# SokhengDin/DNN-MPPI-MPC

Hardware: NVIDIA B200
Metric: mppi_sample_steps_per_sec (higher is better)
Workload: dtype f32

## Files before the change

dnn-mppi-mpc_b200/csrc/mppi_api.cu:

```cuda
#include <cuda_runtime.h>
#include <dlfcn.h>
#include <nccl.h>

#include <algorithm>
#include <cmath>
#include <cstdio>
#include <cstdlib>
#include <cstring>
#include <string>
#include <vector>

#include "mppi_device.cuh"
#include "mppi_launch.h"
#include "mppi_mlp.h"

namespace {

struct NcclApi {
    void *lib = nullptr;
    ncclResult_t (*GetUniqueId)(ncclUniqueId *) = nullptr;
    ncclResult_t (*CommInitRank)(ncclComm_t *, int, ncclUniqueId, int) = nullptr;
    ncclResult_t (*AllGather)(const void *, void *, size_t, ncclDataType_t, ncclComm_t, cudaStream_t) = nullptr;
    ncclResult_t (*CommDestroy)(ncclComm_t) = nullptr;
    const char *(*GetErrorString)(ncclResult_t) = nullptr;
// ... 263 lines not shown
    CKC(cudaSetDevice(c.device));
    cudaDeviceProp prop;
    CKC(cudaGetDeviceProperties(&prop, c.device));
    h->n_sm = prop.multiProcessorCount;
    CKC(cudaStreamCreateWithFlags(&h->stream, cudaStreamNonBlocking));
    h->own_stream = true;

    const int R = c.n_robots, T = c.T, K = c.K;
    int min_cta = 128;
    if (const char *env = std::getenv("MPPI_MIN_CTA_SAMPLES")) min_cta = std::max(32, std::min(MPPI_BLOCK, std::atoi(env)));
    const int chunks = (K + min_cta - 1) / min_cta;
    const int tick_model = (c.model == MPPI_MODEL_DIFFDRIVE_MLP) ? MPPI_MODEL_DIFFDRIVE : c.model;
    h->occ = std::max(1, mppi_tick_occupancy(tick_model, c.collision, c.cost_kind, h->sum, false, c.window, T, false));
    const int occ_stash = mppi_tick_occupancy(tick_model, c.collision, c.cost_kind, h->sum, false, c.window, T, true);
    h->stash = occ_stash >= MPPI_STASH_BLOCKS && c.model != MPPI_MODEL_DIFFDRIVE_MLP;
    int gx = (h->n_sm * h->occ + R - 1) / R;
    gx = std::max(1, std::min(gx, chunks));
    h->grid_x = gx;
    int gxs = (h->n_sm * std::max(1, occ_stash) + R - 1) / R;
    h->grid_x_stash = std::max(1, std::min(gxs, chunks));
    gx = std::max(h->grid_x, h->grid_x_stash);
    {
        const int occ_tpar = (h->sum && c.cost_kind == MPPI_COSTKIND_PATH && c.window != 20 && c.model != MPPI_MODEL_DIFFDRIVE_MLP)
                                 ? mppi_tick_occupancy(tick_model, c.collision, c.cost_kind, true, false, c.window, T, 2) : 0;
        const int gt = std::max(1, std::min(h->n_sm * std::max(1, occ_tpar), (K + 7) / 8));
        const bool fits = occ_tpar >= 1 && (K + gt - 1) / gt <= MPPI_TPAR_SLOTS;
        bool want = R == 1;
        if (const char *env = std::getenv("MPPI_TPAR")) want = std::atoi(env) != 0;
        if (std::getenv("MPPI_VERBOSE"))
            std::fprintf(stderr, "mppi_create: time-parallel rollout: occ %d grid %d fits %d want %d (stash %d sum %d window %d K %d T %d)\n",
                         occ_tpar, gt, (int)fits, (int)want, (int)h->stash, (int)h->sum, c.window, K, T);
        if (want && fits) {
            h->tpar = true;
            h->grid_x_tpar = gt;
            gx = std::max(gx, gt);
        }
        if (std::getenv("MPPI_VERBOSE"))
            std::fprintf(stderr, "mppi_create: rollout path %s, %d CTAs per robot\n", h->tpar ? "tpar" : h->stash ? "stash" : "regenerate",
                         h->tpar ? h->grid_x_tpar : h->stash ? h->grid_x_stash : h->grid_x);
    }

    CKC(gmalloc(h, &h->d_U, sizeof(float) * R * T * 2));
    CKC(cudaMemset(h->d_U, 0, sizeof(float) * R * T * 2));
    CKC(gmalloc(h, &h->d_M, sizeof(float) * T * T));
    CKC(gmalloc(h, &h->d_S, sizeof(float) * (size_t)R * K));
    CKC(gmalloc(h, &h->d_NC, sizeof(int) * (size_t)K));
    const int gmax = (gx + MPPI_MERGE_GROUP_CTAS - 1) / MPPI_MERGE_GROUP_CTAS;
    CKC(gmalloc(h, &h->d_part, sizeof(float) * (size_t)R * (gx + gmax) * MPPI_NF(T)));
    CKC(gmalloc(h, &h->d_out, sizeof(float) * (size_t)R * MPPI_OUT_STRIDE));
    CKC(cudaMemset(h->d_out, 0, sizeof(float) * (size_t)R * MPPI_OUT_STRIDE));
    CKC(gmalloc(h, &h->d_idx, sizeof(int) * R));
    CKC(cudaMemset(h->d_idx, 0, sizeof(int) * R));
    CKC(gmalloc(h, &h->d_ticket, sizeof(unsigned) * (size_t)R * (1 + gmax)));
    CKC(cudaMemset(h->d_ticket, 0, sizeof(unsigned) * (size_t)R * (1 + gmax)));
    CKC(cudaHostAlloc(&h->h_out, sizeof(float) * MPPI_OUT_STRIDE, cudaHostAllocMapped));
    std::memset(h->h_out, 0, sizeof(float) * MPPI_OUT_STRIDE);
    CKC(cudaHostGetDevicePointer(&h->h_out_dev, h->h_out, 0));
    CKC(gmalloc(h, &h->d_first, sizeof(unsigned long long)));
    CKC(cudaHostAlloc(&h->h_first, sizeof(unsigned long long), cudaHostAllocDefault));
    h->idx_mirror = 0; h->idx_mirror_ok = true;
    for (auto &e : h->ev) CKC(cudaEventCreate(&e));
    std::vector<float> M;
    build_filter(T, c.filter_kind, M);
    CKC(cudaMemcpy(h->d_M, M.data(), sizeof(float) * T * T, cudaMemcpyHostToDevice));

    TickArgs &a = h->args;
    std::memset(&a, 0, sizeof(a));
    a.K = K; a.T = T; a.window = c.window; a.yaw_wrap = c.yaw_wrap; a.clamp_nominal = c.clamp_nominal;
    a.k_offset = c.k_offset;
    {
        const double thr = (1.0 - c.param_exploration) * (double)c.K_global;
        long long n = (long long)std::ceil(thr);
        n = std::max(0LL, std::min((long long)c.K_global, n));
        a.n_exploit = (int)n;
    }
    a.dt = (float)c.dt; a.dt_over_L = (float)(c.dt / c.wheel_base);
    a.umax0 = (float)c.u_max[0]; a.umax1 = (float)c.u_max[1];
    for (int i = 0; i < 4; ++i) { a.sw[i] = (float)c.stage_w[i]; a.tw[i] = (float)c.term_w[i]; }
    const double gamma = c.param_lambda * (1.0 - c.param_alpha);
    a.use_gamma = gamma != 0.0;
    a.gq[0] = (float)(gamma * c.sigma[3] / det); a.gq[1] = (float)(-gamma * c.sigma[1] / det);
    a.gq[2] = (float)(-gamma * c.sigma[2] / det); a.gq[3] = (float)(gamma * c.sigma[0] / det);
    const double l00 = std::sqrt(c.sigma[0]), l10 = c.sigma[2] / l00;
    a.chol[0] = (float)l00; a.chol[1] = (float)l10; a.chol[2] = (float)std::sqrt(c.sigma[3] - l10 * l10);
    a.inv_temp = (float)(1.0 / c.temperature);
    for (int i = 0; i < 4; ++i) a.goal[i] = (float)c.goal[i];
    a.ctrl_w[0] = (float)c.ctrl_w[0]; a.ctrl_w[1] = (float)c.ctrl_w[1];
    a.soft_w = (float)c.soft_obs_weight; a.soft_sd = (float)c.soft_obs_safety;
    refresh_obstacle_args(h, nullptr, 0);
    a.U = h->d_U; a.idx = h->d_idx; a.M = h->d_M; a.part = h->d_part; a.ticket = h->d_ticket;
    a.part2 = h->d_part + (size_t)R * gx * MPPI_NF(T); a.ticket2 = h->d_ticket + R; a.merge_gmax = gmax;
    a.out = h->d_out; a.out_host = h->h_out_dev;
    if (c.model == MPPI_MODEL_DIFFDRIVE_MLP) {
        h->mlp = mlp_create(K, T);
        if (!h->mlp) { mppi_destroy(h); return MPPI_E_CUDA; }
    }
#undef CKC
    *out = h;
    return MPPI_OK;
}

int mppi_destroy(mppi_handle_t h) {
    if (!h) return MPPI_E_BADARG;
    cudaSetDevice(h->cfg.device);
    if (h->stream) cudaStreamSynchronize(h->stream);
    if (h->comm && g_nccl.CommDestroy) g_nccl.CommDestroy(h->comm);
    if (h->p2p)
        for (int p = 0; p < h->world; ++p)
            if (p != h->rank && h->peer_buf[p]) cudaIpcCloseMemHandle(h->peer_buf[p]);
    gfree(h, h->d_xchg); gfree(h, h->d_trace); gfree(h, h->d_loop);
    if (h->loop_graph) cudaGraphExecDestroy(h->loop_graph);
    if (h->cap_stream) cudaStreamDestroy(h->cap_stream);
    gfree(h, h->d_paths); gfree(h, h->d_path_len);
    gfree(h, h->d_Sc); gfree(h, h->d_Ssorted); gfree(h, h->d_sorted_idx); gfree(h, h->d_iota); gfree(h, h->d_sort_temp);
    if (h->mlp) mlp_destroy(h->mlp);
    gfree(h, h->d_path); gfree(h, h->d_U); gfree(h, h->d_M); gfree(h, h->d_S); gfree(h, h->d_part);
    gfree(h, h->d_out); gfree(h, h->d_idx); gfree(h, h->d_NC); gfree(h, h->d_ticket); gfree(h, h->d_first);
    gfree(h, h->d_bp_n); gfree(h, h->d_bp_s); gfree(h, h->d_send); gfree(h, h->d_recv); gfree(h, h->d_x0); gfree(h, h->d_opt); gfree(h, h->d_plant_log);
    if (h->h_out) cudaFreeHost(h->h_out);
    if (h->h_first) cudaFreeHost(h->h_first);
    if (h->h_bp_pack) cudaFreeHost(h->h_bp_pack);
    gfree(h, h->d_bp_pack);
    for (auto &e : h->ev) if (e) cudaEventDestroy(e);
    if (h->own_stream && h->stream) cudaStreamDestroy(h->stream);
    delete h;
    return MPPI_OK;
}

int mppi_set_stream(mppi_handle_t h, void *st) {
    if (!h) return MPPI_E_BADARG;
    if (h->own_stream && h->stream) { cudaStreamSynchronize(h->stream); cudaStreamDestroy(h->stream); }
    h->stream = (cudaStream_t)st;
    h->own_stream = false;
    return MPPI_OK;
}

int mppi_synchronize(mppi_handle_t h) {
    if (!h) return MPPI_E_BADARG;
    CK(h, cudaStreamSynchronize(h->stream));
    return check_tick_faults(h);
}

int mppi_set_ref_path(mppi_handle_t h, const double *path, int32_t n, int32_t ncol) {
    if (!h || !path || n < 1 || (ncol != 3 && ncol != 4)) return MPPI_E_BADARG;
    if (h->cfg.model == MPPI_MODEL_BICYCLE && ncol != 4) return fail(h, MPPI_E_BADARG, "bicycle model needs (N,4) path");
    if (h->cfg.cost_kind != MPPI_COSTKIND_PATH) return fail(h, MPPI_E_STATE, "goal / target cost kinds take no reference path");
    CK(h, cudaSetDevice(h->cfg.device));
    CK(h, cudaStreamSynchronize(h->stream));
    std::vector<float4> p((size_t)n);
    for (int i = 0; i < n; ++i) {
        const double *r = path + (size_t)i * ncol;
        p[i] = make_float4((float)r[0], (float)r[1], (float)r[2], ncol == 4 ? (float)r[3] : 0.f);
    }
    gfree(h, h->d_path); h->d_path = nullptr;
    gfree(h, h->d_bp_n); gfree(h, h->d_bp_s); h->d_bp_n = nullptr; h->d_bp_s = nullptr;
    CK(h, gmalloc(h, &h->d_path, sizeof(float4) * n));
    CK(h, cudaMemcpy(h->d_path, p.data(), sizeof(float4) * n, cudaMemcpyHostToDevice));
    CK(h, gmalloc(h, &h->d_bp_n, sizeof(unsigned) * (n + 2)));
    CK(h, gmalloc(h, &h->d_bp_s, sizeof(int) * (n + 2)));
    if (h->strict) {
        gfree(h, h->d_bp_pack); h->d_bp_pack = nullptr;
        if (h->h_bp_pack) { cudaFreeHost(h->h_bp_pack); h->h_bp_pack = nullptr; }
        h->bp_cap = n + 2;
        const size_t bytes = sizeof(unsigned long long) + (sizeof(unsigned) + sizeof(int)) * (size_t)h->bp_cap;
        CK(h, gmalloc(h, &h->d_bp_pack, bytes));
        CK(h, cudaHostAlloc(&h->h_bp_pack, bytes, cudaHostAllocDefault));
    }
// ... 696 lines not shown
```

dnn-mppi-mpc_b200/csrc/mppi_device.cuh:

```cuda
#pragma once
#include <cuda_runtime.h>
#include <stdint.h>
#include <math_constants.h>
#include "../../include/mppi_b200.h"

#ifndef MPPI_DEBUG_CHECKS
#define MPPI_DEBUG_CHECKS 0
#endif
#if MPPI_DEBUG_CHECKS
#include <assert.h>
#define MPPI_DCHECK(c) assert(c)
#else
#define MPPI_DCHECK(c) ((void)0)
#endif
#ifndef MPPI_BLOCK
#define MPPI_BLOCK 256
#endif
#define MPPI_WARPS (MPPI_BLOCK / 32)
#ifndef MPPI_SPT
#define MPPI_SPT 1
#endif
#define MPPI_CHUNK (MPPI_BLOCK * MPPI_SPT)
#ifndef MPPI_MIN_BLOCKS
#define MPPI_MIN_BLOCKS (MPPI_BLOCK >= 512 ? 1 : 768 / MPPI_BLOCK)
#endif
#define MPPI_STASH_BLOCKS (MPPI_BLOCK >= 512 ? 1 : 512 / MPPI_BLOCK)
#define MPPI_PENALTY 1.0e10f
#define MPPI_SENTINEL 1.0e18f
#define MPPI_OUT_HDR 12
#define MPPI_OUT_PEER_TIMEOUT 7
#define MPPI_OUT_FAULT 10
#define MPPI_OUT_STRIDE (MPPI_OUT_HDR + 8 * MPPI_MAX_T)
#define MPPI_OUT_UPRE (MPPI_OUT_HDR + 4 * MPPI_MAX_T)
#define MPPI_OUT_UOLD (MPPI_OUT_HDR + 6 * MPPI_MAX_T)
#define MPPI_NF(T) (4 + 2 * (T))
#define MPPI_MERGE_GROUP_CTAS 16
#define MPPI_NF_MAX MPPI_NF(MPPI_MAX_T)
#define MPPI_XCHG_SLOT(par, r) (((par) * MPPI_MAX_PEERS + (r)) * MPPI_NF_MAX)
#define MPPI_XCHG_WORDS (2 * MPPI_MAX_PEERS * MPPI_NF_MAX)
#define MPPI_XCHG_TRACE 8
#define MPPI_XCHG_BARRIER (MPPI_XCHG_WORDS + MPPI_XCHG_TRACE)
#define MPPI_XCHG_TOTAL (MPPI_XCHG_BARRIER + MPPI_MAX_PEERS)

enum : int {
    F_WRITE_S = 1,
    F_UPDATE = 2,
    F_FROM_S = 4,
    F_HOST_IDX = 8,
    F_TRIPLE_OUT = 16,
    F_KEEP_IDX = 32,
    F_IDX_ONLY = 64,
    F_P2P = 128,
    F_COST_SUM = 0x10000
};

struct TickArgs {
    int K, T, window, n_path, n_obs, yaw_wrap, use_gamma, clamp_nominal;
    int k_offset, n_exploit;
    float dt, dt_over_L, umax0, umax1;
    float sw[4], tw[4];
    float gq[4];
    float chol[3];
    float inv_temp;
    float obs_x[MPPI_MAX_OBSTACLES], obs_y[MPPI_MAX_OBSTACLES];
    float obs_r2[MPPI_MAX_OBSTACLES];
    float obs_far2[MPPI_MAX_OBSTACLES];
    float fp_hl, fp_hw;
    float goal[4];
    float ctrl_w[2];
    float soft_w, soft_sd;
    float obs_vx[MPPI_MAX_OBSTACLES], obs_vy[MPPI_MAX_OBSTACLES];
    float x0[4];
    uint32_t seed_lo, seed_hi, tick;
    int idx_host, flags;
    const float4 *path;
    const int *path_len;
    int path_stride;
    const float *x0_dev;
    float *U;
    int *idx;
    const float *M;
    const float *eps;
    float *S;
    int *NC;
    float *S_user;
    float *part;
    unsigned *ticket;
    float *part2;
    unsigned *ticket2;
    int merge_gmax;
    float *out;
    float *out_host;
    float *u0_out;
    float *triple_out;
    float *plant_state;
    float *plant_log;
    int plant_mode, plant_tick, plant_n;
    unsigned *loop_state;
    unsigned *loop_ticket;
    unsigned long long *peer_buf[MPPI_MAX_PEERS];
    int p2p_rank, p2p_world;
    unsigned p2p_seq;
    unsigned p2p_timeout_ms;
    unsigned long long *trace;
};

__device__ __forceinline__ void philox4x32_10(uint32_t &c0, uint32_t &c1, uint32_t &c2, uint32_t &c3,
                                              uint32_t k0, uint32_t k1) {
#pragma unroll
    for (int r = 0; r < 10; ++r) {
        const uint32_t h0 = __umulhi(0xD2511F53u, c0), l0 = 0xD2511F53u * c0;
        const uint32_t h1 = __umulhi(0xCD9E8D57u, c2), l1 = 0xCD9E8D57u * c2;
        c0 = h1 ^ c1 ^ k0; c1 = l1;
        c2 = h0 ^ c3 ^ k1; c3 = l0;
        k0 += 0x9E3779B9u; k1 += 0xBB67AE85u;
    }
}

__device__ __forceinline__ float u01_open(uint32_t r) {
    return __fadd_rn(__uint_as_float(0x3f800000u | (r >> 9)), -0.99999994f);
}

__device__ __forceinline__ void box_muller(uint32_t ra, uint32_t rb, float &z0, float &z1) {
    const float ua = u01_open(ra), ub = u01_open(rb);
    float rad;
    asm("sqrt.approx.ftz.f32 %0, %1;" : "=f"(rad) : "f"(__fmul_rn(-1.3862943611198906f, __log2f(ua))));
    const float ang = __fmul_rn(6.2831853071795865f, __fadd_rn(ub, -0.5f));
    z0 = __fmul_rn(rad, __cosf(ang));
    z1 = __fmul_rn(rad, __sinf(ang));
}

__device__ __forceinline__ void philox_eps_pair(const TickArgs &a, uint32_t k, uint32_t p, uint32_t robot, float e[4], uint32_t tick_add = 0u) {
    uint32_t c0 = k, c1 = p, c2 = a.tick + tick_add, c3 = robot;
    philox4x32_10(c0, c1, c2, c3, a.seed_lo, a.seed_hi);
    float z0, z1, z2, z3;
    box_muller(c0, c1, z0, z1);
    box_muller(c2, c3, z2, z3);
    e[0] = __fmul_rn(a.chol[0], z0);
    e[1] = __fmaf_rn(a.chol[1], z0, __fmul_rn(a.chol[2], z1));
    e[2] = __fmul_rn(a.chol[0], z2);
    e[3] = __fmaf_rn(a.chol[1], z2, __fmul_rn(a.chol[2], z3));
}

#ifndef MPPI_KEYIDX_SMEM
#define MPPI_KEYIDX_SMEM 1
#endif
struct TickSmem {
    float2 U[MPPI_MAX_T];
    float2 Q[MPPI_MAX_T];
    __align__(16) float wx[MPPI_MAX_WINDOW];
    __align__(16) float wy[MPPI_MAX_WINDOW];
    float2 wyv[MPPI_MAX_WINDOW];
    float x0[4];
    int win_start, n_win16;
    float4 cb[MPPI_MAX_WINDOW / 16];
    __align__(16) float ex[20];
    __align__(16) float ey[20];
    __align__(16) float ec[20];
    float c2x, c2y;
#if MPPI_KEYIDX_SMEM
    __align__(16) float kidx[20];
#endif
};

__device__ __forceinline__ void fill_window_expanded(TickSmem &sm, int nw, int tid, int nthreads) {
    const int jc = nw > 10 ? 10 : nw - 1;
    const float cx = -sm.wx[jc], cy = -sm.wy[jc];
    for (int j = tid; j < 20; j += nthreads) {
        const float wx = __fsub_rn(-sm.wx[j], cx), wy = __fsub_rn(-sm.wy[j], cy);
        const bool valid = j < nw;
        sm.ex[j] = valid ? wx : 0.f;
        sm.ey[j] = valid ? wy : 0.f;
        sm.ec[j] = valid ? __fmaf_rn(wy, wy, __fmul_rn(wx, wx)) : 1e30f;
    }
    if (tid == 0) { sm.c2x = 2.f * cx; sm.c2y = 2.f * cy; }
#if MPPI_KEYIDX_SMEM
    for (int j = tid; j < 20; j += nthreads) sm.kidx[j] = (float)j;
#endif
}

__device__ __forceinline__ float4 chunk_bound(const float *nwx, const float *nwy, int first, int n_valid) {
    float xmin = CUDART_INF_F, xmax = -CUDART_INF_F, ymin = CUDART_INF_F, ymax = -CUDART_INF_F;
#pragma unroll 4
    for (int j = 0; j < n_valid; ++j) {
        const float px = -nwx[first + j], py = -nwy[first + j];
        xmin = fminf(xmin, px); xmax = fmaxf(xmax, px); ymin = fminf(ymin, py); ymax = fmaxf(ymax, py);
    }
    const float cx = 0.5f * (xmin + xmax), cy = 0.5f * (ymin + ymax);
    float r2 = 0.f;
#pragma unroll 4
    for (int j = 0; j < n_valid; ++j) {
        const float dx = -nwx[first + j] - cx, dy = -nwy[first + j] - cy;
        r2 = fmaxf(r2, fmaf(dy, dy, dx * dx));
    }
    return make_float4(cx, cy, sqrtf(r2) * 1.00001f + 1e-6f, 0.f);
}

__device__ __forceinline__ float2 f2_add(float2 a, float2 b) {
    unsigned long long ra = *reinterpret_cast<unsigned long long *>(&a), rb = *reinterpret_cast<unsigned long long *>(&b), rd;
    asm("add.rn.f32x2 %0, %1, %2;" : "=l"(rd) : "l"(ra), "l"(rb));
    return *reinterpret_cast<float2 *>(&rd);
}
__device__ __forceinline__ float2 f2_mul(float2 a, float2 b) {
    unsigned long long ra = *reinterpret_cast<unsigned long long *>(&a), rb = *reinterpret_cast<unsigned long long *>(&b), rd;
    asm("mul.rn.f32x2 %0, %1, %2;" : "=l"(rd) : "l"(ra), "l"(rb));
    return *reinterpret_cast<float2 *>(&rd);
}
__device__ __forceinline__ float2 f2_fma(float2 a, float2 b, float2 c) {
    unsigned long long ra = *reinterpret_cast<unsigned long long *>(&a), rb = *reinterpret_cast<unsigned long long *>(&b),
                       rc = *reinterpret_cast<unsigned long long *>(&c), rd;
    asm("fma.rn.f32x2 %0, %1, %2, %3;" : "=l"(rd) : "l"(ra), "l"(rb), "l"(rc));
    return *reinterpret_cast<float2 *>(&rd);
}

#ifndef MPPI_WP_CHUNK_ILP
#define MPPI_WP_CHUNK_ILP 1
#endif
#ifndef MPPI_WP_FULL
#define MPPI_WP_FULL 0
#endif
#ifndef MPPI_WIN20_EXPANDED
#define MPPI_WIN20_EXPANDED 1
#endif
#ifndef MPPI_ARGMIN_KEY_SEL
#define MPPI_ARGMIN_KEY_SEL 0
#endif
#ifndef MPPI_MIN_TREE
#define MPPI_MIN_TREE 1
#endif
#ifndef MPPI_ARGMIN_PACK
#define MPPI_ARGMIN_PACK 2
#endif
template <int N>
__device__ __forceinline__ float min_tree3(const float (&t)[N]) {
    if constexpr (N == 1) return t[0];
    else if constexpr (N == 2) return fminf(t[0], t[1]);
    else if constexpr (N == 3) return fminf(fminf(t[0], t[1]), t[2]);
    else {
        constexpr int N3 = N / 3, REM = N - 3 * N3, M = N3 + (REM ? 1 : 0);
        float u[M];
#pragma unroll
        for (int i = 0; i < N3; ++i) u[i] = fminf(fminf(t[3 * i], t[3 * i + 1]), t[3 * i + 2]);
        if constexpr (REM == 2) u[N3] = fminf(t[3 * N3], t[3 * N3 + 1]);
        else if constexpr (REM == 1) u[N3] = t[3 * N3];
        return min_tree3<M>(u);
    }
}
template <int CH>
__device__ __forceinline__ void chunk_argmin(const float4 *nwx4, const float4 *nwy4, float x, float y,
                                             float &m_out, float &key_out) {
    const float2 xx = make_float2(x, x), yy = make_float2(y, y);
    float2 d[CH / 2];
#pragma unroll
    for (int q = 0; q < CH / 4; ++q) {
        const float4 X = nwx4[q], Y = nwy4[q];
#if MPPI_ARGMIN_PACK == 2
        const float2 dxa = f2_add(xx, make_float2(X.x, X.y)), dya = f2_add(yy, make_float2(Y.x, Y.y));
        const float2 dxb = f2_add(xx, make_float2(X.z, X.w)), dyb = f2_add(yy, make_float2(Y.z, Y.w));
        d[2 * q] = f2_fma(dya, dya, f2_mul(dxa, dxa));
        d[2 * q + 1] = f2_fma(dyb, dyb, f2_mul(dxb, dxb));
#elif MPPI_ARGMIN_PACK == 1
        const float2 dxa = make_float2(x + X.x, x + X.y), dya = make_float2(y + Y.x, y + Y.y);
        const float2 dxb = make_float2(x + X.z, x + X.w), dyb = make_float2(y + Y.z, y + Y.w);
        d[2 * q] = f2_fma(dya, dya, f2_mul(dxa, dxa));
        d[2 * q + 1] = f2_fma(dyb, dyb, f2_mul(dxb, dxb));
#else
        float dx, dy;
        dx = x + X.x; dy = y + Y.x; d[2 * q].x = fmaf(dy, dy, dx * dx);
        dx = x + X.y; dy = y + Y.y; d[2 * q].y = fmaf(dy, dy, dx * dx);
        dx = x + X.z; dy = y + Y.z; d[2 * q + 1].x = fmaf(dy, dy, dx * dx);
        dx = x + X.w; dy = y + Y.w; d[2 * q + 1].y = fmaf(dy, dy, dx * dx);
#endif
    }
#if MPPI_MIN_TREE
    float m;
    {
        float t[CH / 2];
#pragma unroll
        for (int i = 0; i < CH / 2; ++i) t[i] = fminf(d[i].x, d[i].y);
        m = min_tree3<CH / 2>(t);
    }
#else
    float m = fminf(d[0].x, d[0].y);
#pragma unroll
    for (int i = 1; i < CH / 2; ++i) m = fminf(fminf(m, d[i].x), d[i].y);
#endif
#if MPPI_ARGMIN_KEY_SEL
    {
        float k0 = (float)CH, k1 = (float)CH, k2 = (float)CH, k3 = (float)CH;
#pragma unroll
        for (int i = CH / 8 - 1; i >= 0; --i) {
            const int a0 = i, a1 = i + CH / 8, a2 = i + 2 * (CH / 8), a3 = i + 3 * (CH / 8);
            k0 = d[a0].y == m ? (float)(2 * a0 + 1) : k0; k0 = d[a0].x == m ? (float)(2 * a0) : k0;
            k1 = d[a1].y == m ? (float)(2 * a1 + 1) : k1; k1 = d[a1].x == m ? (float)(2 * a1) : k1;
            k2 = d[a2].y == m ? (float)(2 * a2 + 1) : k2; k2 = d[a2].x == m ? (float)(2 * a2) : k2;
            k3 = d[a3].y == m ? (float)(2 * a3 + 1) : k3; k3 = d[a3].x == m ? (float)(2 * a3) : k3;
        }
        if (CH % 8) {
#pragma unroll
            for (int a = CH / 2 - 1; a >= 4 * (CH / 8); --a) {
                k3 = d[a].y == m ? (float)(2 * a + 1) : k3; k3 = d[a].x == m ? (float)(2 * a) : k3;
            }
#pragma unroll
            for (int a = 4 * (CH / 8) - 1; a >= 3 * (CH / 8); --a) {
                k3 = d[a].y == m ? (float)(2 * a + 1) : k3; k3 = d[a].x == m ? (float)(2 * a) : k3;
            }
        }
        m_out = m;
        key_out = fminf(fminf(k0, k1), fminf(k2, k3));
        return;
    }
#endif
    const float2 nm = make_float2(-m, -m), huge = make_float2(1.2676506e30f, 1.2676506e30f);
#if MPPI_MIN_TREE
    float kt[CH / 2];
#pragma unroll
    for (int i = 0; i < CH / 2; ++i) {
        const float2 k2 = f2_fma(f2_add(d[i], nm), huge, make_float2((float)(2 * i), (float)(2 * i + 1)));
        kt[i] = fminf(k2.x, k2.y);
    }
    m_out = m;
    key_out = min_tree3<CH / 2>(kt);
#else
    float key = CUDART_INF_F;
#pragma unroll
    for (int i = 0; i < CH / 2; ++i) {
#if MPPI_ARGMIN_PACK >= 1
        const float2 k2 = f2_fma(f2_add(d[i], nm), huge, make_float2((float)(2 * i), (float)(2 * i + 1)));
#else
        const float2 k2 = make_float2(fmaf(d[i].x - m, 1.2676506e30f, (float)(2 * i)), fmaf(d[i].y - m, 1.2676506e30f, (float)(2 * i + 1)));
#endif
        key = fminf(fminf(key, k2.x), k2.y);
    }
    m_out = m;
    key_out = key;
#endif
}

template <int WIN>
__device__ __forceinline__ int nearest_wp(const TickSmem &sm, float x, float y) {
    const float4 *nwx4 = reinterpret_cast<const float4 *>(sm.wx);
    const float4 *nwy4 = reinterpret_cast<const float4 *>(sm.wy);
    if (WIN == 20) {
#if MPPI_WIN20_EXPANDED
        const float ax = fmaf(-2.f, x, sm.c2x), ay = fmaf(-2.f, y, sm.c2y);
        const float2 axx = make_float2(ax, ax), ayy = make_float2(ay, ay);
        const float4 *ex4 = reinterpret_cast<const float4 *>(sm.ex), *ey4 = reinterpret_cast<const float4 *>(sm.ey);
        const float4 *ec4 = reinterpret_cast<const float4 *>(sm.ec);
        float2 d[10];
#pragma unroll
        for (int q = 0; q < 5; ++q) {
            const float4 X = ex4[q], Y = ey4[q], C = ec4[q];
            d[2 * q] = f2_fma(make_float2(Y.x, Y.y), ayy, f2_fma(make_float2(X.x, X.y), axx, make_float2(C.x, C.y)));
            d[2 * q + 1] = f2_fma(make_float2(Y.z, Y.w), ayy, f2_fma(make_float2(X.z, X.w), axx, make_float2(C.z, C.w)));
        }
#if MPPI_MIN_TREE
        const float m = fminf(fminf(fminf(fminf(d[0].x, d[0].y), d[1].x), fminf(fminf(d[1].y, d[2].x), d[2].y)),
                              fminf(fminf(fminf(fminf(d[3].x, d[3].y), d[4].x), fminf(fminf(d[4].y, d[5].x), d[5].y)),
                                    fminf(fminf(fminf(fminf(d[6].x, d[6].y), d[7].x), fminf(fminf(d[7].y, d[8].x), d[8].y)),
                                          fminf(d[9].x, d[9].y))));
        const float2 nm = make_float2(-m, -m), huge = make_float2(1.2676506e30f, 1.2676506e30f);
        const float4 *ki4 = reinterpret_cast<const float4 *>(sm.kidx);
        float2 kk[10];
#pragma unroll
        for (int i = 0; i < 10; i += 2) {
            const float4 ki = ki4[i >> 1];
            kk[i] = f2_fma(f2_add(d[i], nm), huge, make_float2(ki.x, ki.y));
            kk[i + 1] = f2_fma(f2_add(d[i + 1], nm), huge, make_float2(ki.z, ki.w));
        }
        const float key = fminf(fminf(fminf(fminf(kk[0].x, kk[0].y), kk[1].x), fminf(fminf(kk[1].y, kk[2].x), kk[2].y)),
                                fminf(fminf(fminf(fminf(kk[3].x, kk[3].y), kk[4].x), fminf(fminf(kk[4].y, kk[5].x), kk[5].y)),
                                      fminf(fminf(fminf(fminf(kk[6].x, kk[6].y), kk[7].x), fminf(fminf(kk[7].y, kk[8].x), kk[8].y)),
                                            fminf(kk[9].x, kk[9].y))));
        return __float2int_rn(key);
#else
        float m = fminf(d[0].x, d[0].y);
#pragma unroll
        for (int i = 1; i < 10; ++i) m = fminf(fminf(m, d[i].x), d[i].y);
        const float2 nm = make_float2(-m, -m), huge = make_float2(1.2676506e30f, 1.2676506e30f);
        float key = CUDART_INF_F;
#if MPPI_KEYIDX_SMEM
        const float4 *ki4 = reinterpret_cast<const float4 *>(sm.kidx);
#pragma unroll
        for (int i = 0; i < 10; i += 2) {
            const float4 ki = ki4[i >> 1];
            const float2 ka = f2_fma(f2_add(d[i], nm), huge, make_float2(ki.x, ki.y));
            const float2 kb = f2_fma(f2_add(d[i + 1], nm), huge, make_float2(ki.z, ki.w));
            key = fminf(fminf(key, ka.x), ka.y);
            key = fminf(fminf(key, kb.x), kb.y);
        }
#else
#pragma unroll
        for (int i = 0; i < 10; ++i) {
            const float2 k2 = f2_fma(f2_add(d[i], nm), huge, make_float2((float)(2 * i), (float)(2 * i + 1)));
            key = fminf(fminf(key, k2.x), k2.y);
        }
#endif
        return __float2int_rn(key);
#endif
#else
        float m, key;
        chunk_argmin<20>(nwx4, nwy4, x, y, m, key);
        return __float2int_rn(key);
#endif
    }
    float bm = CUDART_INF_F, sbm = CUDART_INF_F;
    int bj = 0;
    const int nch = sm.n_win16;
    int c = 0;
#if MPPI_WP_FULL
    for (; c + 3 < nch; c += 4) {
        float m0, k0, m1, k1, m2, k2, m3, k3;
        chunk_argmin<16>(nwx4 + 4 * c, nwy4 + 4 * c, x, y, m0, k0);
        chunk_argmin<16>(nwx4 + 4 * c + 4, nwy4 + 4 * c + 4, x, y, m1, k1);
        chunk_argmin<16>(nwx4 + 4 * c + 8, nwy4 + 4 * c + 8, x, y, m2, k2);
        chunk_argmin<16>(nwx4 + 4 * c + 12, nwy4 + 4 * c + 12, x, y, m3, k3);
        const bool s01 = m1 < m0, s23 = m3 < m2;
        const float ma = s01 ? m1 : m0, mb = s23 ? m3 : m2;
        const float ka = s01 ? k1 + 16.f : k0, kb = s23 ? k3 + 48.f : k2 + 32.f;
        const bool sb = mb < ma;
        const float m = sb ? mb : ma;
        const int j = 16 * c + __float2int_rn(sb ? kb : ka);
        if (m < bm) { bm = m; bj = j; }
    }
    for (; c < nch; ++c) {
        float m, key;
        chunk_argmin<16>(nwx4 + 4 * c, nwy4 + 4 * c, x, y, m, key);
        if (m < bm) { bm = m; bj = 16 * c + __float2int_rn(key); }
    }
    (void)sbm;
    return bj;
#endif
    auto far = [&](int ch) {
        const float4 cb = sm.cb[ch];
        const float ex = x - cb.x, ey = y - cb.y, R = sbm + cb.z;
        return fmaf(ey, ey, ex * ex) > R * R * 1.0002f;
    };
#if MPPI_WP_CHUNK_ILP
    for (; c + 1 < nch; c += 2) {
        if (far(c) && far(c + 1)) continue;
        float m0, k0, m1, k1;
        chunk_argmin<16>(nwx4 + 4 * c, nwy4 + 4 * c, x, y, m0, k0);
        chunk_argmin<16>(nwx4 + 4 * c + 4, nwy4 + 4 * c + 4, x, y, m1, k1);
        const bool second = m1 < m0;
        const float m = second ? m1 : m0;
        const int j = second ? 16 * c + 16 + __float2int_rn(k1) : 16 * c + __float2int_rn(k0);
        if (m < bm) { bm = m; bj = j; sbm = sqrtf(m); }
    }
#endif
    for (; c < nch; ++c) {
        if (far(c)) continue;
        float m, key;
        chunk_argmin<16>(nwx4 + 4 * c, nwy4 + 4 * c, x, y, m, key);
        if (m < bm) { bm = m; bj = 16 * c + __float2int_rn(key); sbm = sqrtf(m); }
    }
    return bj;
}

__device__ __forceinline__ float4 window_ref(const TickSmem &sm, int j) {
    MPPI_DCHECK(j >= 0 && j < MPPI_MAX_WINDOW);
    const float2 yv = sm.wyv[j];
    return make_float4(-sm.wx[j], -sm.wy[j], yv.x, yv.y);
}

__device__ __forceinline__ void sincos_cw(float x, float &s, float &c) {
    const float t = fmaf(x, 0.636619772f, 12582912.f);
    const int q = __float_as_int(t);
    const float k = t - 12582912.f;
    float r = fmaf(k, -1.5707963705062866f, x);
    r = fmaf(k, 4.371138828673793e-08f, r);
    r = fmaf(k, 1.7151245100058819e-15f, r);
    const float r2 = r * r;
    float sp = fmaf(r2, -1.9515295891e-4f, 8.3321608736e-3f);
    sp = fmaf(sp, r2, -1.6666654611e-1f);
    sp = fmaf(sp * r2, r, r);
    float cp = fmaf(r2, 2.443315711809948e-5f, -1.388731625493765e-3f);
    cp = fmaf(cp, r2, 4.166664568298827e-2f);
    cp = fmaf(cp, r2, -0.5f);
    cp = fmaf(cp, r2, 1.0f);
    const float ss = (q & 1) ? cp : sp, cc = (q & 1) ? sp : cp;
    s = __int_as_float(__float_as_int(ss) ^ ((q << 30) & 0x80000000));
    c = __int_as_float(__float_as_int(cc) ^ (((q + 1) << 30) & 0x80000000));
}

__device__ __forceinline__ float wrap_2pi(float yaw) {
    const float b = 6.2831855f;
    const float y2 = yaw + b;
    const float q = floorf(y2 * 0.15915494f);
    float r = fmaf(-q, b, y2);
    if (r < 0.f) r += b;
    if (r >= b) r -= b;
    return r;
}

template <int MODEL, int COLL>
__device__ __forceinline__ bool collided(const TickArgs &a, float x, float y, float cs, float sn) {
    bool hit = false;
    if constexpr (COLL == MPPI_COLLISION_NONE) {
        return false;
    } else if constexpr (COLL == MPPI_COLLISION_CIRCLE) {
        for (int m = 0; m < a.n_obs; ++m) {
            const float dx = x - a.obs_x[m], dy = y - a.obs_y[m];
            hit |= (dx * dx + dy * dy < a.obs_r2[m]);
        }
        return hit;
    } else {
    for (int m = 0; m < a.n_obs; ++m) {
        const float ox = a.obs_x[m], oy = a.obs_y[m];
        const float cx = x - ox, cy = y - oy;
        if (cx * cx + cy * cy >= a.obs_far2[m]) continue;
        const float r2 = a.obs_r2[m];
        const float ac = a.fp_hl * cs, as = a.fp_hl * sn, bc = a.fp_hw * cs, bs = a.fp_hw * sn;
        float px, py;
        px = cx - ac;      py = cy - as;      hit |= (px * px + py * py < r2);
        px = cx - ac - bs; py = cy - as + bc; hit |= (px * px + py * py < r2);
        px = cx - bs;      py = cy + bc;      hit |= (px * px + py * py < r2);
        px = cx + ac - bs; py = cy + as + bc; hit |= (px * px + py * py < r2);
        px = cx + ac;      py = cy + as;      hit |= (px * px + py * py < r2);
        px = cx + ac + bs; py = cy + as - bc; hit |= (px * px + py * py < r2);
        px = cx + bs;      py = cy - bc;      hit |= (px * px + py * py < r2);
        px = cx - ac + bs; py = cy - as - bc; hit |= (px * px + py * py < r2);
    }
    return hit;
    }
}

template <int MODEL>
__device__ __forceinline__ float tracking_cost(const float4 ref, const float z[4], float yaw_eff, const float w[4]) {
    const float dx = z[0] - ref.x, dy = z[1] - ref.y, dyaw = yaw_eff - ref.z;
    float c = w[0] * dx * dx + w[1] * dy * dy + w[2] * dyaw * dyaw;
    if (MODEL == MPPI_MODEL_BICYCLE) { const float dv = z[3] - ref.w; c += w[3] * dv * dv; }
    return c;
}

#define MPPI_WIN_GOAL (-1)
#define MPPI_WIN_TARGET (-2)

__device__ __forceinline__ float goal_cost(const TickArgs &a, const float z[4], const float w[4]) {
    const float dx = z[0] - a.goal[0], dy = z[1] - a.goal[1];
    const float d2 = fmaf(dy, dy, dx * dx);
    const float diff = atan2f(dy, dx) - z[2];
    const float k = rintf(diff * 0.15915494309189535f);
    float r = fmaf(k, -6.2831854820251465f, diff);
    r = fmaf(k, 1.7484555314695172e-07f, r);
    return w[0] * d2 + w[1] * r * r;
}

__device__ __forceinline__ float target_soft_cost(const TickArgs &a, const float z[4], float v0, float v1, int t,
                                                  const float w[4], bool full) {
    const float ex = z[0] - a.goal[0], ey = z[1] - a.goal[1], eth = z[2] - a.goal[2];
    float c = w[0] * ex * ex + w[1] * ey * ey + w[2] * eth * eth;
    if (full) {
        c += a.ctrl_w[0] * v0 * v0 + a.ctrl_w[1] * v1 * v1;
        const float tt = (float)t * a.dt;
        float soft = 0.f;
        for (int m = 0; m < a.n_obs; ++m) {
            const float dx = z[0] - fmaf(a.obs_vx[m], tt, a.obs_x[m]), dy = z[1] - fmaf(a.obs_vy[m], tt, a.obs_y[m]);
            const float d = sqrtf(fmaf(dy, dy, dx * dx));
            if (d < a.soft_sd) soft += expf(a.soft_sd - d);
        }
        c = fmaf(a.soft_w, soft, c);
    }
    return c;
}

template <int MODEL, int WIN>
__device__ __forceinline__ float eval_state_cost(const TickArgs &a, const TickSmem &sm, const float z[4], float v0, float v1,
                                                 int t, const float w[4], float4 &ref, float &yaw_eff) {
    if constexpr (WIN == MPPI_WIN_GOAL) {
        return goal_cost(a, z, w);
    } else if constexpr (WIN == MPPI_WIN_TARGET) {
        return target_soft_cost(a, z, v0, v1, t, w, true);
    } else {
        const int j = nearest_wp<WIN>(sm, z[0], z[1]);
        ref = window_ref(sm, j);
        yaw_eff = (MODEL == MPPI_MODEL_BICYCLE && a.yaw_wrap) ? wrap_2pi(z[2]) : z[2];
        return tracking_cost<MODEL>(ref, z, yaw_eff, w);
    }
}
template <int MODEL, int WIN>
__device__ __forceinline__ float eval_terminal_cost(const TickArgs &a, const float z[4], const float4 ref, float yaw_eff) {
    if constexpr (WIN == MPPI_WIN_GOAL) return goal_cost(a, z, a.tw);
    else if constexpr (WIN == MPPI_WIN_TARGET) return target_soft_cost(a, z, 0.f, 0.f, 0, a.tw, false);
    else return tracking_cost<MODEL>(ref, z, yaw_eff, a.tw);
}

template <int MODEL>
__device__ __forceinline__ void dyn_step(const TickArgs &a, float z[4], float v0, float v1, float cs, float sn) {
    if (MODEL == MPPI_MODEL_BICYCLE) {
        const float vel = z[3];
        z[0] += vel * cs * a.dt;
        z[1] += vel * sn * a.dt;
        z[2] += vel * a.dt_over_L * tanf(v0);
        z[3] += v1 * a.dt;
    } else {
        z[0] += v0 * cs * a.dt;
        z[1] += v0 * sn * a.dt;
        z[2] += v1 * a.dt;
    }
}

template <int MODEL>
__device__ __forceinline__ void dyn_step_tan(const TickArgs &a, float z[4], float v0, float v1, float cs, float sn, float tan_v0) {
    if (MODEL == MPPI_MODEL_BICYCLE) {
        const float vel = z[3];
        z[0] += vel * cs * a.dt;
        z[1] += vel * sn * a.dt;
        z[2] += vel * a.dt_over_L * tan_v0;
        z[3] += v1 * a.dt;
    } else {
        dyn_step<MODEL>(a, z, v0, v1, cs, sn);
    }
}

__device__ __forceinline__ float clampf(float v, float lim) { return fminf(fmaxf(v, -lim), lim); }

template <int MODEL, int COLL, bool SUM, bool INJ, int WIN, int SPT>
__device__ __forceinline__ void rollout_samples(const TickArgs &a, const TickSmem &sm, const uint32_t (&kg)[SPT], const int (&klocal)[SPT],
                                                uint32_t robot, const bool (&exploit)[SPT], float2 *stash, float (&smooth)[SPT], int (&ncoll)[SPT],
                                                uint32_t tick_add = 0u) {
    const int T = a.T;
    float z[SPT][4], cs[SPT], sn[SPT], acc[SPT], v0[SPT], v1[SPT], yaw_eff[SPT];
    int nc[SPT];
    float4 ref[SPT];
    bool hit[SPT];
    const float2 *eps_k[SPT];
#pragma unroll
    for (int s = 0; s < SPT; ++s) {
        z[s][0] = sm.x0[0]; z[s][1] = sm.x0[1]; z[s][2] = sm.x0[2]; z[s][3] = sm.x0[3];
        sincos_cw(z[s][2], sn[s], cs[s]);
        acc[s] = 0.f; nc[s] = 0; v0[s] = v1[s] = 0.f; yaw_eff[s] = 0.f; hit[s] = false;
        ref[s] = make_float4(0.f, 0.f, 0.f, 0.f);
        eps_k[s] = INJ ? reinterpret_cast<const float2 *>(a.eps) + (size_t)klocal[s] * T : nullptr;
    }

    auto fetch = [&](int s, int tp, float e[4]) {
        if (INJ) {
            e[0] = e[1] = e[2] = e[3] = 0.f;
            if (tp < T) { const float2 ea = eps_k[s][tp]; e[0] = ea.x; e[1] = ea.y; }
            if (tp + 1 < T) { const float2 eb = eps_k[s][tp + 1]; e[2] = eb.x; e[3] = eb.y; }
        } else {
            philox_eps_pair(a, kg[s], (uint32_t)(tp >> 1), robot, e, tick_add);
        }
    };
    auto step = [&](int s, int t, float e0, float e1) {
        MPPI_DCHECK(t >= 0 && t < T);
        if (stash) stash[t * MPPI_CHUNK + s * MPPI_BLOCK] = make_float2(e0, e1);
        const float2 u = sm.U[t];
        v0[s] = clampf(exploit[s] ? __fadd_rn(u.x, e0) : e0, a.umax0);
        v1[s] = clampf(exploit[s] ? __fadd_rn(u.y, e1) : e1, a.umax1);
        dyn_step<MODEL>(a, z[s], v0[s], v1[s], cs[s], sn[s]);
        sincos_cw(z[s][2], sn[s], cs[s]);
        if (SUM) {
            const float c = eval_state_cost<MODEL, WIN>(a, sm, z[s], v0[s], v1[s], t, a.sw, ref[s], yaw_eff[s]);
            const float2 q = sm.Q[t];
            acc[s] += c + (q.x * v0[s] + q.y * v1[s]);
            hit[s] = collided<MODEL, COLL>(a, z[s][0], z[s][1], cs[s], sn[s]);
            nc[s] += hit[s] ? 1 : 0;
        }
    };

    float e[SPT][4];
#pragma unroll
    for (int s = 0; s < SPT; ++s) fetch(s, 0, e[s]);
    const int n_fetch_pairs = WIN >= 0 ? (T - 1) >> 1 : T >> 1;
    int tp = 0;
    for (int i = 0; i < n_fetch_pairs; ++i, tp += 2) {
        float en[SPT][4];
#pragma unroll
        for (int s = 0; s < SPT; ++s) fetch(s, tp + 2, en[s]);
#pragma unroll
        for (int s = 0; s < SPT; ++s) step(s, tp, e[s][0], e[s][1]);
#pragma unroll
        for (int s = 0; s < SPT; ++s) step(s, tp + 1, e[s][2], e[s][3]);
#pragma unroll
        for (int s = 0; s < SPT; ++s) { e[s][0] = en[s][0]; e[s][1] = en[s][1]; e[s][2] = en[s][2]; e[s][3] = en[s][3]; }
    }
#pragma unroll
    for (int s = 0; s < SPT; ++s) {
        if (WIN >= 0) {
            step(s, tp, e[s][0], e[s][1]);
            if (!(T & 1)) step(s, tp + 1, e[s][2], e[s][3]);
        } else if (T & 1) {
            step(s, T - 1, e[s][0], e[s][1]);
        }
        if (SUM) {
            acc[s] += eval_terminal_cost<MODEL, WIN>(a, z[s], ref[s], yaw_eff[s]);
            nc[s] += hit[s] ? 1 : 0;
        } else {
            const float2 q = sm.Q[T - 1];
            acc[s] = eval_state_cost<MODEL, WIN>(a, sm, z[s], v0[s], v1[s], T - 1, a.sw, ref[s], yaw_eff[s]) + (q.x * v0[s] + q.y * v1[s]);
            acc[s] += eval_terminal_cost<MODEL, WIN>(a, z[s], ref[s], yaw_eff[s]);
            nc[s] = collided<MODEL, COLL>(a, z[s][0], z[s][1], cs[s], sn[s]) ? 2 : 0;
        }
        smooth[s] = acc[s];
        ncoll[s] = nc[s];
    }
}

#define MPPI_TPAR_SLOTS 64
#ifndef MPPI_TPAR_PROBE
#define MPPI_TPAR_PROBE 0
#endif
#if MPPI_TPAR_PROBE
#include <cstdio>
#endif
struct TparSmem {
    int prog[MPPI_TPAR_SLOTS / 32];
    int next;
};
template <int MODEL, int COLL, int WIN>
__device__ __forceinline__ void rollout_tpar(const TickArgs &a, const TickSmem &sm, TparSmem &ts, const int k_begin, const int n, const uint32_t robot,
                                             float2 *stash, float4 *zbuf, float &smooth, int &ncoll, const uint32_t tick_add) {
    const int T = a.T, tid = threadIdx.x;
    const uint32_t inv_n = n > 1 ? (uint32_t)((0x100000000ull + (uint32_t)n - 1u) / (uint32_t)n) : 0u;
    auto div_n = [&](int i) { return n > 1 ? (int)__umulhi((uint32_t)i, inv_n) : i; };
    if (tid < MPPI_TPAR_SLOTS / 32) ts.prog[tid] = 0;
    if (tid == 0) ts.next = 0;
    const uint32_t kg0 = (uint32_t)(a.k_offset + k_begin);
    MPPI_DCHECK(n >= 1 && n <= MPPI_TPAR_SLOTS && MPPI_TPAR_SLOTS <= MPPI_BLOCK);
#if MPPI_TPAR_PROBE
    long long pc[5];
#define MPPI_TPAR_STAMP(i) pc[i] = clock64()
#else
#define MPPI_TPAR_STAMP(i)
#endif
    MPPI_TPAR_STAMP(0);
    {
        const int npairs = (T + 1) >> 1, items = n * npairs;
        for (int i = tid; i < items; i += MPPI_BLOCK) {
            const int p = div_n(i), slot = i - p * n;
            MPPI_DCHECK(p == i / n && 2 * p < T && slot >= 0 && slot < n);
            float e[4];
            philox_eps_pair(a, kg0 + (uint32_t)slot, (uint32_t)p, robot, e, tick_add);
            stash[(2 * p) * MPPI_TPAR_SLOTS + slot] = make_float2(e[0], e[1]);
            if (2 * p + 1 < T) stash[(2 * p + 1) * MPPI_TPAR_SLOTS + slot] = make_float2(e[2], e[3]);
            if (MODEL == MPPI_MODEL_BICYCLE) {
                const bool exploit = (int)(kg0 + (uint32_t)slot) < a.n_exploit;
                const float ua = sm.U[2 * p].x, ub = (2 * p + 1 < T) ? sm.U[2 * p + 1].x : 0.f;
// ... 105 lines not shown
```

Measured before the change: 125.4 billion.

## Vectorize noise generation, dynamics and cost math with packed f32x2 instructions

Rewrites the Box-Muller noise path, the Cholesky scaling, the sincos polynomial, the unicycle dynamics step, the tracking cost and the WIN20 distance setup to use paired f32x2 add/mul/fma PTX instructions. It also reorders the chol array and aligns it to 8 bytes so two entries load as a float2. The goal is to halve the FP32 instruction count in the ALU-bound rollout loop. In exchange it adds register packing and moves, and rounding changes slightly (for example an fma replaces a separate mul and add in dynamics), so outputs may not match bit for bit.

```diff
diff --git a/dnn-mppi-mpc_b200/csrc/mppi_api.cu b/dnn-mppi-mpc_b200/csrc/mppi_api.cu
--- a/dnn-mppi-mpc_b200/csrc/mppi_api.cu
+++ b/dnn-mppi-mpc_b200/csrc/mppi_api.cu
@@ -369,7 +369,7 @@
     a.gq[0] = (float)(gamma * c.sigma[3] / det); a.gq[1] = (float)(-gamma * c.sigma[1] / det);
     a.gq[2] = (float)(-gamma * c.sigma[2] / det); a.gq[3] = (float)(gamma * c.sigma[0] / det);
     const double l00 = std::sqrt(c.sigma[0]), l10 = c.sigma[2] / l00;
-    a.chol[0] = (float)l00; a.chol[1] = (float)l10; a.chol[2] = (float)std::sqrt(c.sigma[3] - l10 * l10);
+    a.chol[0] = (float)l00; a.chol[1] = (float)std::sqrt(c.sigma[3] - l10 * l10); a.chol[2] = (float)l10;
     a.inv_temp = (float)(1.0 / c.temperature);
     for (int i = 0; i < 4; ++i) a.goal[i] = (float)c.goal[i];
     a.ctrl_w[0] = (float)c.ctrl_w[0]; a.ctrl_w[1] = (float)c.ctrl_w[1];
diff --git a/dnn-mppi-mpc_b200/csrc/mppi_device.cuh b/dnn-mppi-mpc_b200/csrc/mppi_device.cuh
--- a/dnn-mppi-mpc_b200/csrc/mppi_device.cuh
+++ b/dnn-mppi-mpc_b200/csrc/mppi_device.cuh
@@ -60,7 +60,7 @@
     float dt, dt_over_L, umax0, umax1;
     float sw[4], tw[4];
     float gq[4];
-    float chol[3];
+    __align__(8) float chol[3];
     float inv_temp;
     float obs_x[MPPI_MAX_OBSTACLES], obs_y[MPPI_MAX_OBSTACLES];
     float obs_r2[MPPI_MAX_OBSTACLES];
@@ -105,6 +105,23 @@
     unsigned long long *trace;
 };
 
+__device__ __forceinline__ float2 f2_add(float2 a, float2 b) {
+    unsigned long long ra = *reinterpret_cast<unsigned long long *>(&a), rb = *reinterpret_cast<unsigned long long *>(&b), rd;
+    asm("add.rn.f32x2 %0, %1, %2;" : "=l"(rd) : "l"(ra), "l"(rb));
+    return *reinterpret_cast<float2 *>(&rd);
+}
+__device__ __forceinline__ float2 f2_mul(float2 a, float2 b) {
+    unsigned long long ra = *reinterpret_cast<unsigned long long *>(&a), rb = *reinterpret_cast<unsigned long long *>(&b), rd;
+    asm("mul.rn.f32x2 %0, %1, %2;" : "=l"(rd) : "l"(ra), "l"(rb));
+    return *reinterpret_cast<float2 *>(&rd);
+}
+__device__ __forceinline__ float2 f2_fma(float2 a, float2 b, float2 c) {
+    unsigned long long ra = *reinterpret_cast<unsigned long long *>(&a), rb = *reinterpret_cast<unsigned long long *>(&b),
+                       rc = *reinterpret_cast<unsigned long long *>(&c), rd;
+    asm("fma.rn.f32x2 %0, %1, %2, %3;" : "=l"(rd) : "l"(ra), "l"(rb), "l"(rc));
+    return *reinterpret_cast<float2 *>(&rd);
+}
+
 __device__ __forceinline__ void philox4x32_10(uint32_t &c0, uint32_t &c1, uint32_t &c2, uint32_t &c3,
                                               uint32_t k0, uint32_t k1) {
 #pragma unroll
@@ -117,29 +134,34 @@
     }
 }
 
-__device__ __forceinline__ float u01_open(uint32_t r) {
-    return __fadd_rn(__uint_as_float(0x3f800000u | (r >> 9)), -0.99999994f);
-}
-
-__device__ __forceinline__ void box_muller(uint32_t ra, uint32_t rb, float &z0, float &z1) {
-    const float ua = u01_open(ra), ub = u01_open(rb);
-    float rad;
-    asm("sqrt.approx.ftz.f32 %0, %1;" : "=f"(rad) : "f"(__fmul_rn(-1.3862943611198906f, __log2f(ua))));
-    const float ang = __fmul_rn(6.2831853071795865f, __fadd_rn(ub, -0.5f));
-    z0 = __fmul_rn(rad, __cosf(ang));
-    z1 = __fmul_rn(rad, __sinf(ang));
+__device__ __forceinline__ float2 u01_open2(uint32_t r, uint32_t s) {
+    return f2_add(make_float2(__uint_as_float(0x3f800000u | (r >> 9)), __uint_as_float(0x3f800000u | (s >> 9))),
+                  make_float2(-0.99999994f, -0.99999994f));
+}
+
+__device__ __forceinline__ float lg2_normal(float x) {
+    float y;
+    asm("lg2.approx.ftz.f32 %0, %1;" : "=f"(y) : "f"(x));
+    return y;
 }
 
 __device__ __forceinline__ void philox_eps_pair(const TickArgs &a, uint32_t k, uint32_t p, uint32_t robot, float e[4], uint32_t tick_add = 0u) {
     uint32_t c0 = k, c1 = p, c2 = a.tick + tick_add, c3 = robot;
     philox4x32_10(c0, c1, c2, c3, a.seed_lo, a.seed_hi);
-    float z0, z1, z2, z3;
-    box_muller(c0, c1, z0, z1);
-    box_muller(c2, c3, z2, z3);
-    e[0] = __fmul_rn(a.chol[0], z0);
-    e[1] = __fmaf_rn(a.chol[1], z0, __fmul_rn(a.chol[2], z1));
-    e[2] = __fmul_rn(a.chol[0], z2);
-    e[3] = __fmaf_rn(a.chol[1], z2, __fmul_rn(a.chol[2], z3));
+    const float2 ua = u01_open2(c0, c2), ub = u01_open2(c1, c3);
+    const float2 l = f2_mul(make_float2(lg2_normal(ua.x), lg2_normal(ua.y)), make_float2(-1.3862943611198906f, -1.3862943611198906f));
+    float rad0, rad1;
+    asm("sqrt.approx.ftz.f32 %0, %1;" : "=f"(rad0) : "f"(l.x));
+    asm("sqrt.approx.ftz.f32 %0, %1;" : "=f"(rad1) : "f"(l.y));
+    const float2 ang = f2_mul(make_float2(6.2831853071795865f, 6.2831853071795865f), f2_add(ub, make_float2(-0.5f, -0.5f)));
+    const float2 z01 = f2_mul(make_float2(rad0, rad0), make_float2(__cosf(ang.x), __sinf(ang.x)));
+    const float2 z23 = f2_mul(make_float2(rad1, rad1), make_float2(__cosf(ang.y), __sinf(ang.y)));
+    const float2 ld = make_float2(a.chol[0], a.chol[1]);
+    const float2 p01 = f2_mul(z01, ld), p23 = f2_mul(z23, ld);
+    e[0] = p01.x;
+    e[1] = __fmaf_rn(a.chol[2], z01.x, p01.y);
+    e[2] = p23.x;
+    e[3] = __fmaf_rn(a.chol[2], z23.x, p23.y);
 }
 
 #ifndef MPPI_KEYIDX_SMEM
@@ -194,23 +216,6 @@
         r2 = fmaxf(r2, fmaf(dy, dy, dx * dx));
     }
     return make_float4(cx, cy, sqrtf(r2) * 1.00001f + 1e-6f, 0.f);
-}
-
-__device__ __forceinline__ float2 f2_add(float2 a, float2 b) {
-    unsigned long long ra = *reinterpret_cast<unsigned long long *>(&a), rb = *reinterpret_cast<unsigned long long *>(&b), rd;
-    asm("add.rn.f32x2 %0, %1, %2;" : "=l"(rd) : "l"(ra), "l"(rb));
-    return *reinterpret_cast<float2 *>(&rd);
-}
-__device__ __forceinline__ float2 f2_mul(float2 a, float2 b) {
-    unsigned long long ra = *reinterpret_cast<unsigned long long *>(&a), rb = *reinterpret_cast<unsigned long long *>(&b), rd;
-    asm("mul.rn.f32x2 %0, %1, %2;" : "=l"(rd) : "l"(ra), "l"(rb));
-    return *reinterpret_cast<float2 *>(&rd);
-}
-__device__ __forceinline__ float2 f2_fma(float2 a, float2 b, float2 c) {
-    unsigned long long ra = *reinterpret_cast<unsigned long long *>(&a), rb = *reinterpret_cast<unsigned long long *>(&b),
-                       rc = *reinterpret_cast<unsigned long long *>(&c), rd;
-    asm("fma.rn.f32x2 %0, %1, %2, %3;" : "=l"(rd) : "l"(ra), "l"(rb), "l"(rc));
-    return *reinterpret_cast<float2 *>(&rd);
 }
 
 #ifndef MPPI_WP_CHUNK_ILP
@@ -343,8 +348,8 @@
     const float4 *nwy4 = reinterpret_cast<const float4 *>(sm.wy);
     if (WIN == 20) {
 #if MPPI_WIN20_EXPANDED
-        const float ax = fmaf(-2.f, x, sm.c2x), ay = fmaf(-2.f, y, sm.c2y);
-        const float2 axx = make_float2(ax, ax), ayy = make_float2(ay, ay);
+        const float2 axy = f2_fma(make_float2(-2.f, -2.f), make_float2(x, y), make_float2(sm.c2x, sm.c2y));
+        const float2 axx = make_float2(axy.x, axy.x), ayy = make_float2(axy.y, axy.y);
         const float4 *ex4 = reinterpret_cast<const float4 *>(sm.ex), *ey4 = reinterpret_cast<const float4 *>(sm.ey);
         const float4 *ec4 = reinterpret_cast<const float4 *>(sm.ec);
         float2 d[10];
@@ -466,18 +471,16 @@
 __device__ __forceinline__ void sincos_cw(float x, float &s, float &c) {
     const float t = fmaf(x, 0.636619772f, 12582912.f);
     const int q = __float_as_int(t);
-    const float k = t - 12582912.f;
+    const float k = __fsub_rn(t, 12582912.f);
     float r = fmaf(k, -1.5707963705062866f, x);
     r = fmaf(k, 4.371138828673793e-08f, r);
     r = fmaf(k, 1.7151245100058819e-15f, r);
-    const float r2 = r * r;
-    float sp = fmaf(r2, -1.9515295891e-4f, 8.3321608736e-3f);
-    sp = fmaf(sp, r2, -1.6666654611e-1f);
-    sp = fmaf(sp * r2, r, r);
-    float cp = fmaf(r2, 2.443315711809948e-5f, -1.388731625493765e-3f);
-    cp = fmaf(cp, r2, 4.166664568298827e-2f);
-    cp = fmaf(cp, r2, -0.5f);
-    cp = fmaf(cp, r2, 1.0f);
+    const float r2 = __fmul_rn(r, r);
+    const float2 rr = make_float2(r2, r2);
+    float2 p = make_float2(fmaf(r2, -1.9515295891e-4f, 8.3321608736e-3f), fmaf(r2, 2.443315711809948e-5f, -1.388731625493765e-3f));
+    p = f2_fma(p, rr, make_float2(-1.6666654611e-1f, 4.166664568298827e-2f));
+    p = f2_fma(p, rr, make_float2(-0.f, -0.5f));
+    const float sp = fmaf(p.x, r, r), cp = fmaf(p.y, r2, 1.0f);
     const float ss = (q & 1) ? cp : sp, cc = (q & 1) ? sp : cp;
     s = __int_as_float(__float_as_int(ss) ^ ((q << 30) & 0x80000000));
     c = __int_as_float(__float_as_int(cc) ^ (((q + 1) << 30) & 0x80000000));
@@ -527,8 +530,10 @@
 
 template <int MODEL>
 __device__ __forceinline__ float tracking_cost(const float4 ref, const float z[4], float yaw_eff, const float w[4]) {
-    const float dx = z[0] - ref.x, dy = z[1] - ref.y, dyaw = yaw_eff - ref.z;
-    float c = w[0] * dx * dx + w[1] * dy * dy + w[2] * dyaw * dyaw;
+    const float2 d = f2_add(make_float2(z[0], z[1]), make_float2(-ref.x, -ref.y));
+    const float2 wd = f2_mul(make_float2(w[0], w[1]), d);
+    const float dyaw = __fsub_rn(yaw_eff, ref.z);
+    float c = fmaf(__fmul_rn(w[2], dyaw), dyaw, fmaf(wd.x, d.x, __fmul_rn(wd.y, d.y)));
     if (MODEL == MPPI_MODEL_BICYCLE) { const float dv = z[3] - ref.w; c += w[3] * dv * dv; }
     return c;
 }
@@ -594,9 +599,9 @@
         z[2] += vel * a.dt_over_L * tanf(v0);
         z[3] += v1 * a.dt;
     } else {
-        z[0] += v0 * cs * a.dt;
-        z[1] += v0 * sn * a.dt;
-        z[2] += v1 * a.dt;
+        const float2 xy = f2_fma(f2_mul(make_float2(cs, sn), make_float2(v0, v0)), make_float2(a.dt, a.dt), make_float2(z[0], z[1]));
+        z[0] = xy.x; z[1] = xy.y;
+        z[2] = fmaf(v1, a.dt, z[2]);
     }
 }
 
@@ -654,7 +659,7 @@
         if (SUM) {
             const float c = eval_state_cost<MODEL, WIN>(a, sm, z[s], v0[s], v1[s], t, a.sw, ref[s], yaw_eff[s]);
             const float2 q = sm.Q[t];
-            acc[s] += c + (q.x * v0[s] + q.y * v1[s]);
+            acc[s] = __fadd_rn(acc[s], __fadd_rn(c, fmaf(q.x, v0[s], __fmul_rn(q.y, v1[s]))));
             hit[s] = collided<MODEL, COLL>(a, z[s][0], z[s][1], cs[s], sn[s]);
             nc[s] += hit[s] ? 1 : 0;
         }
```

New measurement: 128.2 billion, median of 6. 1.02x the previous value.
